# linkedin/ml-ease

Hardware: NVIDIA H100
Metric: ADMM iterations/sec (higher is better)
Workload: dtype f32 data / f64 reductions / bf16 (dense) or e4m3 (CSR) Gram operands

## Files before the change

ml-ease_b200/csrc/k3_cholesky.cu:

```cuda
#include <algorithm>
#include <cstdlib>

#include "kernels.cuh"

namespace mlease {

constexpr int NB = 32;
constexpr int TB = 64;

__global__ void chol_prep_kernel(const Problem* __restrict__ probs, int share) {
  const Problem& pb = probs[blockIdx.z];
  const float* __restrict__ hpart = share > 1 ? probs[blockIdx.z - blockIdx.z % share].Hpart : pb.Hpart;
  Ctrl* c = pb.ctrl;
  if (c->done || !c->need_hess) return;
  const int ldh = pb.ldh, Dt = pb.Dt, Dp = pb.Dp, S = pb.gram_slices;
  const int i = blockIdx.y * blockDim.y + threadIdx.y;
  const int j = blockIdx.x * blockDim.x + threadIdx.x;
  if (i >= ldh || j >= ldh || j > i) return;
  double v;
  if (i < Dt) {
    double s = 0.0;
    const size_t off = (size_t)i * Dp + j;
    for (int t = 0; t < S; t++) s += (double)hpart[(size_t)t * Dp * Dp + off];
    s *= (double)pb.gram_unscale;
    if (i == j) s += pb.q[i];
    v = s;
  } else {
    v = (i == j) ? 1.0 : 0.0;
  }
  pb.Lc[(size_t)i * ldh + j] = v;
}

constexpr int RB = 64;
__global__ void __launch_bounds__(32) chol_diag_kernel(const Problem* __restrict__ probs, int k) {
  const Problem& pb = probs[blockIdx.x];
  Ctrl* c = pb.ctrl;
  if (c->done || !c->need_hess) return;
  __shared__ double A[NB][NB + 1];
  const int ldh = pb.ldh;
  const int c0 = k * NB;
  const double* H = pb.Lc;
  const int lane = threadIdx.x;
  double a[NB];
#pragma unroll
  for (int kk = 0; kk < NB; kk++) a[kk] = (kk <= lane) ? H[(size_t)(c0 + lane) * ldh + c0 + kk] : 0.0;
  int bad = 0;
  double dinv[NB];
#pragma unroll
  for (int j = 0; j < NB; j++) {
    double djj = __shfl_sync(0xffffffffu, a[j], j);
    if (!(djj > 0.0)) { bad = 1; djj = 1.0; }
    const double r = rsqrt(djj);
    dinv[j] = r;
    if (lane == j) a[j] = djj * r;
    else if (lane > j) a[j] = a[j] * r;
#pragma unroll
    for (int kk = j + 1; kk < NB; kk++) {
      const double lkj = __shfl_sync(0xffffffffu, a[j], kk);
      if (lane >= kk) a[kk] -= a[j] * lkj;
    }
  }
#pragma unroll
  for (int kk = 0; kk < NB; kk++) {
    A[lane][kk] = (kk <= lane) ? a[kk] : 0.0;
    pb.Ldiag[(size_t)(c0 + lane) * NB + kk] = (kk <= lane) ? a[kk] : 0.0;
  }
  __syncwarp();
  {
    const int cc = lane;
    double li[NB];
#pragma unroll
    for (int i = 0; i < NB; i++) {
      double sacc = 0.0;
#pragma unroll
      for (int kk = 0; kk < NB; kk++)
        if (kk < i) sacc += A[i][kk] * li[kk];
      li[i] = i < cc ? 0.0 : (i == cc ? dinv[i] : -sacc * dinv[i]);
    }
#pragma unroll
    for (int i = 0; i < NB; i++) pb.Ldinv[(size_t)(c0 + i) * NB + cc] = li[i];
  }
  if (lane == 0 && bad) c->fail = 1;
}

__global__ void __launch_bounds__(256) chol_panel_kernel(const Problem* __restrict__ probs, int k) {
  const Problem& pb = probs[blockIdx.y];
  Ctrl* c = pb.ctrl;
  if (c->done || !c->need_hess) return;
  __shared__ double Li[NB][NB + 1];
  __shared__ double P[RB][NB + 1];
  const int ldh = pb.ldh;
  const int c0 = k * NB;
  double* H = pb.Lc;
  const int tid = threadIdx.x;
  const int r0 = c0 + NB + blockIdx.x * RB;
  if (r0 >= ldh) return;
  const int rows = min(RB, ldh - r0);
  for (int e = tid; e < NB * NB; e += 256) Li[e / NB][e % NB] = pb.Ldinv[(size_t)(c0 + e / NB) * NB + e % NB];
  for (int e = tid; e < rows * NB; e += 256) {
    const int i = e / NB, j = e % NB;
    P[i][j] = H[(size_t)(r0 + i) * ldh + c0 + j];
  }
  __syncthreads();
  for (int e = tid; e < rows * NB; e += 256) {
    const int i = e / NB, j = e % NB;
    double sacc = 0.0;
    for (int kk = 0; kk <= j; kk++) sacc += P[i][kk] * Li[j][kk];
    H[(size_t)(r0 + i) * ldh + c0 + j] = sacc;
  }
}

__global__ void __launch_bounds__(256) chol_update_kernel(const Problem* __restrict__ probs, int k, int jlimit) {
  const Problem& pb = probs[blockIdx.z];
  Ctrl* c = pb.ctrl;
  if (c->done || !c->need_hess) return;
  if (blockIdx.x > blockIdx.y) return;
  const int ldh = pb.ldh;
  const int base = (k + 1) * NB;
  const int i0 = base + blockIdx.y * TB, j0 = base + blockIdx.x * TB;
  if (i0 >= ldh || j0 >= ldh || j0 >= jlimit) return;
  __shared__ double Ai[NB][TB + 2];
  __shared__ double Aj[NB][TB + 2];
  double* H = pb.Lc;
  const int c0 = k * NB;
  const int tid = threadIdx.x;
  for (int e = tid; e < TB * NB; e += 256) {
    const int i = e / NB, kk = e % NB;
    Ai[kk][i] = (i0 + i < ldh) ? H[(size_t)(i0 + i) * ldh + c0 + kk] : 0.0;
    Aj[kk][i] = (j0 + i < ldh) ? H[(size_t)(j0 + i) * ldh + c0 + kk] : 0.0;
  }
  __syncthreads();
  const int ti = (tid / 16) * 4, tj = (tid % 16) * 4;
  double acc[4][4];
#pragma unroll
  for (int a = 0; a < 4; a++)
#pragma unroll
    for (int b = 0; b < 4; b++) acc[a][b] = 0.0;
#pragma unroll 4
  for (int kk = 0; kk < NB; kk++) {
    double x[4], y[4];
#pragma unroll
    for (int a = 0; a < 4; a++) { x[a] = Ai[kk][ti + a]; y[a] = Aj[kk][tj + a]; }
#pragma unroll
    for (int a = 0; a < 4; a++)
#pragma unroll
      for (int b = 0; b < 4; b++) acc[a][b] += x[a] * y[b];
  }
#pragma unroll
  for (int a = 0; a < 4; a++)
#pragma unroll
    for (int b = 0; b < 4; b++) {
      const int i = i0 + ti + a, j = j0 + tj + b;
      if (i < ldh && j <= i && j < jlimit) H[(size_t)i * ldh + j] -= acc[a][b];
    }
}

__global__ void chol_finish_kernel(const Problem* __restrict__ probs) {
  const Problem& pb = probs[blockIdx.y];
  Ctrl* c = pb.ctrl;
  if (c->done || !c->need_hess) return;
  const int c0 = blockIdx.x * NB;
  for (int e = threadIdx.x; e < NB * NB; e += blockDim.x) {
    const int i = e / NB, j = e % NB;
    if (j <= i) pb.Lc[(size_t)(c0 + i) * pb.ldh + c0 + j] = pb.Ldiag[(size_t)(c0 + i) * NB + j];
  }
  if (threadIdx.x == 0 && blockIdx.x == 0) {
    if (c->fail == 1) { c->done = 1; c->hess_valid = 0; }
    else { c->hess_valid = 1; c->hess_builds++; c->tot_hess++; c->bfgs_count = 0; c->h0_scale = 1.0; c->build_step = c->newton_steps; c->ysym_use = pb.Ysym; }
  }
}

template <int NR>
__global__ void __launch_bounds__(256) trinv_kernel(const Problem* __restrict__ probs, int leaf) {
  const Problem& pb = probs[blockIdx.y];
  Ctrl* c = pb.ctrl;
  if (c->done || !c->need_hess) return;
  constexpr int CPT = NR / 8;
  __shared__ double Lt[NB][NB + 1];
  __shared__ double Yt[NB][NR + 2];
  __shared__ double Rb[NB][NR + 2];
  const int ldh = pb.ldh;
  const int c0 = blockIdx.x * NR;
  if (c0 >= ldh) return;
  const int nb = leaf > 0 ? min(ldh, (c0 / leaf + 1) * leaf) / NB : ldh / NB;
  const int ncols = min(NR, ldh - c0);
  const int kb0 = c0 / NB;
  const int tid = threadIdx.x;
  const int ti = tid >> 3, tq = tid & 7;
  const double* __restrict__ L = pb.Lc;
  double* __restrict__ Y = pb.Yinv;
  const int lr = tid >> 3, lc = (tid & 7) * 4;
  for (int kb = kb0; kb < nb; kb++) {
// ... 21 lines not shown
        const double l = Lt[ti][kk];
#pragma unroll
        for (int q = 0; q < CPT; q++) acc[q] -= l * Yt[kk][tq + 8 * q];
      }
      __syncthreads();
    }
#pragma unroll
    for (int q = 0; q < CPT; q++) Rb[ti][tq + 8 * q] = acc[q];
#pragma unroll
    for (int q = 0; q < 4; q++) Lt[lr][lc + q] = pb.Ldinv[(size_t)(r0 + lr) * NB + lc + q];
    __syncthreads();
    double yv[CPT];
#pragma unroll
    for (int q = 0; q < CPT; q++) yv[q] = 0.0;
    for (int kk = 0; kk <= ti; kk++) {
      const double l = Lt[ti][kk];
#pragma unroll
      for (int q = 0; q < CPT; q++) yv[q] += l * Rb[kk][tq + 8 * q];
    }
#pragma unroll
    for (int q = 0; q < CPT; q++)
      if (tq + 8 * q < ncols) Y[(size_t)(r0 + ti) * ldh + c0 + tq + 8 * q] = yv[q];
    __syncthreads();
  }
}

__global__ void __launch_bounds__(256) hinv_syrk_kernel(const Problem* __restrict__ probs) {
  const Problem& pb = probs[blockIdx.z];
  Ctrl* c = pb.ctrl;
  if (c->done || !c->need_hess) return;
  if (blockIdx.x > blockIdx.y) return;
  const int ldh = pb.ldh;
  const int i0 = blockIdx.y * TB, j0 = blockIdx.x * TB;
  if (i0 >= ldh) return;
  __shared__ double Yi[NB][TB + 1];
  __shared__ double Yj[NB][TB + 1];
  const double* Y = pb.Yinv;
  const int tid = threadIdx.x;
  const int ti = (tid / 16) * 4, tj = (tid % 16) * 4;
  double acc[4][4];
#pragma unroll
  for (int a = 0; a < 4; a++)
#pragma unroll
    for (int b = 0; b < 4; b++) acc[a][b] = 0.0;
  for (int k0 = (i0 / NB) * NB; k0 < ldh; k0 += NB) {
    for (int e = tid; e < NB * TB; e += 256) {
      const int kk = e / TB, cc = e % TB;
      const int k = k0 + kk;
      Yi[kk][cc] = (i0 + cc < ldh && i0 + cc <= k) ? Y[(size_t)k * ldh + i0 + cc] : 0.0;
      Yj[kk][cc] = (j0 + cc < ldh && j0 + cc <= k) ? Y[(size_t)k * ldh + j0 + cc] : 0.0;
    }
    __syncthreads();
#pragma unroll 4
    for (int kk = 0; kk < NB; kk++) {
      double x[4], y[4];
#pragma unroll
      for (int a = 0; a < 4; a++) { x[a] = Yi[kk][ti + a]; y[a] = Yj[kk][tj + a]; }
#pragma unroll
      for (int a = 0; a < 4; a++)
#pragma unroll
        for (int b = 0; b < 4; b++) acc[a][b] += x[a] * y[b];
    }
    __syncthreads();
  }
#pragma unroll
  for (int a = 0; a < 4; a++)
#pragma unroll
    for (int b = 0; b < 4; b++) {
      const int i = i0 + ti + a, j = j0 + tj + b;
      if (i < ldh && j < ldh) {
        pb.Hinv[(size_t)i * ldh + j] = acc[a][b];
        pb.Hinv[(size_t)j * ldh + i] = acc[a][b];
      }
    }
}


constexpr int WNB = 256;
constexpr int WLEAF = 256;
constexpr int DM = 128, DN = 64, DK = 16;
constexpr int DA_SZ = DM * 20 > DK * (DM + 4) ? DM * 20 : DK * (DM + 4);
constexpr int DB_SZ = DN * 20 > DK * (DN + 4) ? DN * 20 : DK * (DN + 4);
constexpr size_t DGEMM_SMEM = (size_t)2 * (DA_SZ + DB_SZ) * sizeof(double);

__device__ __forceinline__ void dmma_8x8x4(double& c0, double& c1, double a, double b) {
  asm volatile("mma.sync.aligned.m8n8k4.row.col.f64.f64.f64.f64 {%0,%1}, {%2}, {%3}, {%0,%1};" : "+d"(c0), "+d"(c1) : "d"(a), "d"(b));
}

template <bool A_KC, bool B_KC>
__global__ void __launch_bounds__(256, 2) dgemm_kernel(const Problem* __restrict__ probs, int mode, int p0, int p1) {
  const Problem& pb = probs[blockIdx.z];
  Ctrl* ctl = pb.ctrl;
  if (ctl->done || !ctl->need_hess) return;
  const int ldh = pb.ldh;
  const double* A; const double* B; double* C;
  int M, N, K;
  if (mode == 0) {
    const int c = p0, w = p1;
    M = N = ldh - c - w; K = w;
    A = B = pb.Lc + (size_t)(c + w) * ldh + c;
    C = pb.Lc + (size_t)(c + w) * ldh + (c + w);
  } else if (mode == 1 || mode == 2) {
    const int m = p0, r0 = 2 * blockIdx.y * m;
    const int m2 = min(m, ldh - r0 - m);
    if (m2 <= 0) return;
    M = m2; N = m;
    if (mode == 1) {
      K = m;
      A = pb.Lc + (size_t)(r0 + m) * ldh + r0;
      B = pb.Yinv + (size_t)r0 * ldh + r0;
      C = pb.Hinv + (size_t)(r0 + m) * ldh + r0;
    } else {
      K = m2;
      A = pb.Yinv + (size_t)(r0 + m) * ldh + (r0 + m);
      B = pb.Hinv + (size_t)(r0 + m) * ldh + r0;
      C = pb.Yinv + (size_t)(r0 + m) * ldh + r0;
    }
  } else {
    M = N = K = ldh;
    A = B = pb.Yinv;
    C = pb.Hinv;
  }
  const int tiles_n = (N + DN - 1) / DN;
  const int i0 = (blockIdx.x / tiles_n) * DM, j0 = (blockIdx.x % tiles_n) * DN;
  if (i0 >= M) return;
  if ((mode == 0 || mode == 3) && j0 >= i0 + DM) return;
  int klo = 0, khi = K;
  if (mode == 1) klo = j0;
  if (mode == 2) khi = min(K, i0 + DM);
  if (mode == 3) klo = max(i0, j0);

  extern __shared__ double dg_smem[];
  double* As = dg_smem;
  double* Bs = dg_smem + 2 * DA_SZ;
  const int tid = threadIdx.x, warp = tid >> 5, lane = tid & 31;
  const int g = lane >> 2, tg = lane & 3;
  const int wm = (warp & 3) * 32, wn = (warp >> 2) * 32;

  double2 ra[4], rb[2];
  auto gload = [&](int k0) {
#pragma unroll
    for (int q = 0; q < 4; q++) {
      if (A_KC) {
        const int row = (tid >> 3) + 32 * q, kk = (tid & 7) * 2;
        ra[q] = (i0 + row < M) ? *reinterpret_cast<const double2*>(A + (size_t)(i0 + row) * ldh + k0 + kk) : make_double2(0.0, 0.0);
      } else {
        const int kk = (tid >> 6) + 4 * q, ii = (tid & 63) * 2;
        ra[q] = (i0 + ii < M) ? *reinterpret_cast<const double2*>(A + (size_t)(k0 + kk) * ldh + i0 + ii) : make_double2(0.0, 0.0);
      }
    }
#pragma unroll
    for (int q = 0; q < 2; q++) {
      if (B_KC) {
        const int col = (tid >> 3) + 32 * q, kk = (tid & 7) * 2;
        rb[q] = (j0 + col < N) ? *reinterpret_cast<const double2*>(B + (size_t)(j0 + col) * ldh + k0 + kk) : make_double2(0.0, 0.0);
      } else {
        const int kk = (tid >> 5) + 8 * q, jj = (tid & 31) * 2;
        rb[q] = (j0 + jj < N) ? *reinterpret_cast<const double2*>(B + (size_t)(k0 + kk) * ldh + j0 + jj) : make_double2(0.0, 0.0);
      }
    }
  };
  auto sstore = [&](int buf) {
    double* a = As + buf * DA_SZ;
    double* b = Bs + buf * DB_SZ;
#pragma unroll
    for (int q = 0; q < 4; q++) {
      if (A_KC) *reinterpret_cast<double2*>(a + ((tid >> 3) + 32 * q) * 20 + (tid & 7) * 2) = ra[q];
      else *reinterpret_cast<double2*>(a + ((tid >> 6) + 4 * q) * (DM + 4) + (tid & 63) * 2) = ra[q];
    }
#pragma unroll
    for (int q = 0; q < 2; q++) {
      if (B_KC) *reinterpret_cast<double2*>(b + ((tid >> 3) + 32 * q) * 20 + (tid & 7) * 2) = rb[q];
      else *reinterpret_cast<double2*>(b + ((tid >> 5) + 8 * q) * (DN + 4) + (tid & 31) * 2) = rb[q];
    }
  };

  double acc[4][4][2];
#pragma unroll
  for (int a = 0; a < 4; a++)
#pragma unroll
    for (int b = 0; b < 4; b++) acc[a][b][0] = acc[a][b][1] = 0.0;

  if (klo < khi) {
    gload(klo);
    sstore(0);
    __syncthreads();
    int buf = 0;
    for (int k0 = klo; k0 < khi; k0 += DK) {
      const bool more = k0 + DK < khi;
      if (more) gload(k0 + DK);
      const double* a = As + buf * DA_SZ;
      const double* b = Bs + buf * DB_SZ;
#pragma unroll
      for (int k4 = 0; k4 < DK; k4 += 4) {
        double fa[4], fb[4];
#pragma unroll
        for (int f = 0; f < 4; f++) {
          fa[f] = A_KC ? a[(wm + f * 8 + g) * 20 + k4 + tg] : a[(k4 + tg) * (DM + 4) + wm + f * 8 + g];
          fb[f] = B_KC ? b[(wn + f * 8 + g) * 20 + k4 + tg] : b[(k4 + tg) * (DN + 4) + wn + f * 8 + g];
        }
#pragma unroll
        for (int fm = 0; fm < 4; fm++)
#pragma unroll
          for (int fn = 0; fn < 4; fn++) dmma_8x8x4(acc[fm][fn][0], acc[fm][fn][1], fa[fm], fb[fn]);
      }
      if (more) sstore(buf ^ 1);
      __syncthreads();
      buf ^= 1;
    }
  }

#pragma unroll
  for (int fm = 0; fm < 4; fm++) {
    const int i = i0 + wm + fm * 8 + g;
    if (i >= M) continue;
#pragma unroll
    for (int fn = 0; fn < 4; fn++) {
      const int j = j0 + wn + fn * 8 + 2 * tg;
      if (j >= N) continue;
      const double v0 = acc[fm][fn][0], v1 = acc[fm][fn][1];
      if (mode == 0) {
        double* d = C + (size_t)i * ldh + j;
        if (j + 1 <= i) { double2 o = *reinterpret_cast<double2*>(d); o.x -= v0; o.y -= v1; *reinterpret_cast<double2*>(d) = o; }
        else if (j <= i) d[0] -= v0;
      } else if (mode == 1) {
        *reinterpret_cast<double2*>(C + (size_t)i * ldh + j) = make_double2(v0, v1);
      } else if (mode == 2) {
        *reinterpret_cast<double2*>(C + (size_t)i * ldh + j) = make_double2(-v0, -v1);
      } else {
        if (j <= i) { C[(size_t)i * ldh + j] = v0; C[(size_t)j * ldh + i] = v0; }
        if (j + 1 <= i) { C[(size_t)i * ldh + j + 1] = v1; C[(size_t)(j + 1) * ldh + i] = v1; }
      }
    }
  }
}

template <bool A_KC, bool B_KC>
static cudaError_t dgemm_launch(const Problem* d_probs, int nprob, int mode, int p0, int p1, int M, int N, int nmerge, cudaStream_t st,
                                int* launches) {
  {
    static bool configured[64] = {};
    int dev = 0;
    cudaGetDevice(&dev);
    if (dev < 0 || dev >= 64 || !configured[dev]) {
      cudaError_t e = cudaFuncSetAttribute(dgemm_kernel<A_KC, B_KC>, cudaFuncAttributeMaxDynamicSharedMemorySize, (int)DGEMM_SMEM);
      if (e != cudaSuccess) return e;
      if (dev >= 0 && dev < 64) configured[dev] = true;
    }
  }
  const int tiles = ((M + DM - 1) / DM) * ((N + DN - 1) / DN);
  if (tiles <= 0 || nmerge <= 0) return cudaSuccess;
  dgemm_kernel<A_KC, B_KC><<<dim3(tiles, nmerge, nprob), 256, DGEMM_SMEM, st>>>(d_probs, mode, p0, p1);
  if (launches) *launches += 1;
  return cudaGetLastError();
}

constexpr int TM = 128, TN = 128, TK = 16;
constexpr int TA_LD = TK + 4, TB_LD = TN + 8;
constexpr int TA_SZ = TM * TA_LD, TB_SZ = TK * TB_LD;

__device__ __forceinline__ uint32_t to_tf32(double x) {
  uint32_t r;
  const float f = (float)x;
  asm("cvt.rna.tf32.f32 %0, %1;" : "=r"(r) : "f"(f));
  return r;
}
__device__ __forceinline__ void mma_tf32_16x8x8(float (&c)[4], const uint32_t (&a)[4], const uint32_t (&b)[2]) {
  asm volatile("mma.sync.aligned.m16n8k8.row.col.f32.tf32.tf32.f32 {%0,%1,%2,%3}, {%4,%5,%6,%7}, {%8,%9}, {%0,%1,%2,%3};"
               : "+f"(c[0]), "+f"(c[1]), "+f"(c[2]), "+f"(c[3])
               : "r"(a[0]), "r"(a[1]), "r"(a[2]), "r"(a[3]), "r"(b[0]), "r"(b[1]));
}

__global__ void __launch_bounds__(256, 2) merge_tf32_kernel(const Problem* __restrict__ probs, int mode, int m) {
  const Problem& pb = probs[blockIdx.z];
  Ctrl* ctl = pb.ctrl;
  if (ctl->done || !ctl->need_hess) return;
  const int ldh = pb.ldh;
  const int r0 = 2 * blockIdx.y * m;
  const int m2 = min(m, ldh - r0 - m);
  if (m2 <= 0) return;
  const int M = m2, N = m;
  const double* __restrict__ A; const double* __restrict__ B; double* __restrict__ C;
  int K;
  if (mode == 1) {
    K = m;
    A = pb.Lc + (size_t)(r0 + m) * ldh + r0;
    B = pb.Yinv + (size_t)r0 * ldh + r0;
    C = pb.Hinv + (size_t)(r0 + m) * ldh + r0;
  } else {
    K = m2;
    A = pb.Yinv + (size_t)(r0 + m) * ldh + (r0 + m);
    B = pb.Hinv + (size_t)(r0 + m) * ldh + r0;
    C = pb.Yinv + (size_t)(r0 + m) * ldh + r0;
  }
  const int tiles_n = (N + TN - 1) / TN;
  const int i0 = (blockIdx.x / tiles_n) * TM, j0 = (blockIdx.x % tiles_n) * TN;
  if (i0 >= M) return;
  int klo = 0, khi = K;
  if (mode == 1) klo = j0;
  else khi = min(K, i0 + TM);

  __shared__ __align__(16) uint32_t As[2][TA_SZ];
  __shared__ __align__(16) uint32_t Bs[2][TB_SZ];
  const int tid = threadIdx.x, warp = tid >> 5, lane = tid & 31;
  const int g = lane >> 2, tg = lane & 3;
  const int wm = (warp & 1) * 64, wn = (warp >> 1) * 32;

  const double* pa = A + (size_t)(i0 + (tid >> 3)) * ldh + klo + (tid & 7) * 2;
  const double* pbk = B + (size_t)(klo + (tid >> 6)) * ldh + j0 + (tid & 63) * 2;
  const size_t a_step = (size_t)32 * ldh, b_step = (size_t)4 * ldh, b_adv = (size_t)TK * ldh;
  unsigned a_ok = 0;
#pragma unroll
  for (int q = 0; q < 4; q++) a_ok |= (i0 + (tid >> 3) + 32 * q < M ? 1u : 0u) << q;
  const bool b_ok = j0 + (tid & 63) * 2 < N;
  double2 ra[4], rb[4];
  auto gload = [&]() {
#pragma unroll
    for (int q = 0; q < 4; q++)
      ra[q] = ((a_ok >> q) & 1u) ? __ldg(reinterpret_cast<const double2*>(pa + q * a_step)) : make_double2(0.0, 0.0);
#pragma unroll
    for (int q = 0; q < 4; q++)
      rb[q] = b_ok ? __ldg(reinterpret_cast<const double2*>(pbk + q * b_step)) : make_double2(0.0, 0.0);
    pa += TK;
    pbk += b_adv;
  };
  auto sstore = [&](int buf) {
#pragma unroll
    for (int q = 0; q < 4; q++) {
      const int row = (tid >> 3) + 32 * q, kk = (tid & 7) * 2;
      *reinterpret_cast<uint2*>(&As[buf][row * TA_LD + kk]) = make_uint2(to_tf32(ra[q].x), to_tf32(ra[q].y));
    }
#pragma unroll
    for (int q = 0; q < 4; q++) {
      const int kk = (tid >> 6) + 4 * q, jj = (tid & 63) * 2;
      *reinterpret_cast<uint2*>(&Bs[buf][kk * TB_LD + jj]) = make_uint2(to_tf32(rb[q].x), to_tf32(rb[q].y));
    }
// ... 12 lines not shown
    sstore(0);
    __syncthreads();
    int buf = 0;
    for (int k0 = klo; k0 < khi; k0 += TK) {
      const bool more = k0 + TK < khi;
      if (more) gload();
      const uint32_t* a = As[buf];
      const uint32_t* b = Bs[buf];
#pragma unroll
      for (int k8 = 0; k8 < TK; k8 += 8) {
        uint32_t fa[4][4], fb[4][2];
#pragma unroll
        for (int f = 0; f < 4; f++) {
          const uint32_t* pa = a + (wm + f * 16 + g) * TA_LD + k8 + tg;
          fa[f][0] = pa[0];
          fa[f][1] = pa[8 * TA_LD];
          fa[f][2] = pa[4];
          fa[f][3] = pa[8 * TA_LD + 4];
          const uint32_t* pbk = b + (k8 + tg) * TB_LD + wn + f * 8 + g;
          fb[f][0] = pbk[0];
          fb[f][1] = pbk[4 * TB_LD];
        }
#pragma unroll
        for (int fm = 0; fm < 4; fm++)
#pragma unroll
          for (int fn = 0; fn < 4; fn++) mma_tf32_16x8x8(acc[fm][fn], fa[fm], fb[fn]);
      }
      if (more) sstore(buf ^ 1);
      __syncthreads();
      buf ^= 1;
    }
  }

  const double sgn = mode == 1 ? 1.0 : -1.0;
#pragma unroll
  for (int fm = 0; fm < 4; fm++)
#pragma unroll
    for (int h = 0; h < 2; h++) {
      const int i = i0 + wm + fm * 16 + g + 8 * h;
      if (i >= M) continue;
#pragma unroll
      for (int fn = 0; fn < 4; fn++) {
        const int j = j0 + wn + fn * 8 + 2 * tg;
        if (j >= N) continue;
        *reinterpret_cast<double2*>(C + (size_t)i * ldh + j) =
            make_double2(sgn * (double)acc[fm][fn][2 * h], sgn * (double)acc[fm][fn][2 * h + 1]);
      }
    }
}

static cudaError_t merge_tf32_launch(const Problem* d_probs, int nprob, int mode, int m, int nmerge, cudaStream_t st, int* launches) {
  const int t = (m + TM - 1) / TM;
  if (t <= 0 || nmerge <= 0) return cudaSuccess;
  merge_tf32_kernel<<<dim3(t * ((m + TN - 1) / TN), nmerge, nprob), 256, 0, st>>>(d_probs, mode, m);
  if (launches) *launches += 1;
  return cudaGetLastError();
}
constexpr int CHOL_WIDE_MIN = 1000;

__global__ void __launch_bounds__(256) ysym_kernel(const Problem* __restrict__ probs) {
  const Problem& pb = probs[blockIdx.z];
  const Ctrl* c = pb.ctrl;
  if (c->done || !c->need_hess) return;
  const int bi = blockIdx.y, bj = blockIdx.x;
  if (bj > bi) return;
  __shared__ float t[32][33];
  const int ldh = pb.ldh;
  const int tx = threadIdx.x & 31, ty = threadIdx.x >> 5;
  for (int r = ty; r < 32; r += 8) {
    const int i = bi * 32 + r, j = bj * 32 + tx;
    const float v = j <= i ? (float)pb.Yinv[(size_t)i * ldh + j] : 0.f;
    t[r][tx] = v;
    if (j <= i) pb.Ysym[(size_t)i * ldh + j] = __float2bfloat16_rn(v);
  }
  __syncthreads();
  for (int r = ty; r < 32; r += 8) {
    const int j = bj * 32 + r, i = bi * 32 + tx;
    if (j < i) pb.Ysym[(size_t)j * ldh + i] = __float2bfloat16_rn(t[tx][r]);
  }
}

bool cholesky_factored_direction(int ldh) { return ldh > 2048; }

static cudaError_t cholesky_launch_wide(const Problem* d_probs, int nprob, int ldh, cudaStream_t st, int* launches, bool factored_direction) {
  cudaError_t e;
  for (int c = 0; c < ldh; c += WNB) {
    const int w = std::min(WNB, ldh - c);
    for (int k = c / NB; k < (c + w) / NB; k++) {
      const int below = ldh - (k + 1) * NB;
      const int gx = below > 0 ? (below + RB - 1) / RB : 1;
      chol_diag_kernel<<<nprob, 32, 0, st>>>(d_probs, k);
      if (below > 0) chol_panel_kernel<<<dim3(gx, nprob), 256, 0, st>>>(d_probs, k);
      if (launches) *launches += 2;
      const int inner = c + w - (k + 1) * NB;
      if (inner > 0) {
        chol_update_kernel<<<dim3((inner + TB - 1) / TB, (below + TB - 1) / TB, nprob), 256, 0, st>>>(d_probs, k, c + w);
        if (launches) *launches += 1;
      }
    }
    const int rest = ldh - c - w;
    if (rest > 0 && (e = dgemm_launch<true, true>(d_probs, nprob, 0, c, w, rest, rest, 1, st, launches)) != cudaSuccess) return e;
  }
  trinv_kernel<64><<<dim3((ldh + 63) / 64, nprob), 256, 0, st>>>(d_probs, WLEAF);
  if ((e = cudaGetLastError()) != cudaSuccess) return e;
  if (launches) *launches += 1;
  for (int m = WLEAF; m < ldh; m *= 2) {
    const int nmerge = (ldh + 2 * m - 1) / (2 * m);
    if (factored_direction) {
      if ((e = merge_tf32_launch(d_probs, nprob, 1, m, nmerge, st, launches)) != cudaSuccess) return e;
      if ((e = merge_tf32_launch(d_probs, nprob, 2, m, nmerge, st, launches)) != cudaSuccess) return e;
      continue;
    }
    if ((e = dgemm_launch<true, false>(d_probs, nprob, 1, m, 0, m, m, nmerge, st, launches)) != cudaSuccess) return e;
    if ((e = dgemm_launch<true, false>(d_probs, nprob, 2, m, 0, m, m, nmerge, st, launches)) != cudaSuccess) return e;
  }
  if (factored_direction) {
    ysym_kernel<<<dim3(ldh / 32, ldh / 32, nprob), 256, 0, st>>>(d_probs);
    if (launches) *launches += 1;
    return cudaGetLastError();
  }
  return dgemm_launch<false, false>(d_probs, nprob, 3, 0, 0, ldh, ldh, 1, st, launches);
}

__global__ void chol_share_begin_kernel(const Problem* __restrict__ probs, int nprob, int share) {
  const int b = blockIdx.x * blockDim.x + threadIdx.x;
  if (b < nprob && b % share != 0) probs[b].ctrl->need_hess = 0;
}
__global__ void chol_share_end_kernel(const Problem* __restrict__ probs, int nprob, int share) {
  const int b = blockIdx.x * blockDim.x + threadIdx.x;
  if (b >= nprob || b % share == 0) return;
  Ctrl* c = probs[b].ctrl;
  const Ctrl* lead = probs[b - b % share].ctrl;
  c->need_hess = 1;
  if (lead->fail == 1) { c->fail = 1; c->done = 1; c->hess_valid = 0; }
  else {
    c->hess_valid = 1; c->hess_builds++; c->tot_hess++; c->bfgs_count = 0; c->h0_scale = 1.0; c->build_step = c->newton_steps;
    c->ysym_use = probs[b - b % share].Ysym;
  }
}
__device__ __forceinline__ int detach_owner(const Problem* __restrict__ probs, int nprob, int b) {
  const Problem& pb = probs[b];
  const Ctrl* c = pb.ctrl;
  const void* use = c->ysym_use;
  if (!use || use == (const void*)pb.Ysym || (!c->done && c->need_hess)) return -1;
  for (int j = 0; j < nprob; j++) {
    if ((const void*)probs[j].Ysym != use) continue;
    const Ctrl* oc = probs[j].ctrl;
    return (!oc->done && oc->need_hess) ? j : -1;
  }
  return -1;
}
__global__ void __launch_bounds__(256) ysym_detach_kernel(const Problem* __restrict__ probs, int nprob, int mode) {
  if (mode == 1) {
    const int b = blockIdx.x * blockDim.x + threadIdx.x;
    if (b < nprob && detach_owner(probs, nprob, b) >= 0) probs[b].ctrl->ysym_use = probs[b].Ysym;
    return;
  }
  const int b = blockIdx.y;
  const int o = detach_owner(probs, nprob, b);
  if (o < 0) return;
  const size_t n16 = (size_t)probs[b].ldh * probs[b].ldh / 8;
  const uint4* __restrict__ src = reinterpret_cast<const uint4*>(probs[o].Ysym);
  uint4* __restrict__ dst = reinterpret_cast<uint4*>(probs[b].Ysym);
  for (size_t e = (size_t)blockIdx.x * blockDim.x + threadIdx.x; e < n16; e += (size_t)gridDim.x * blockDim.x) dst[e] = src[e];
}
cudaError_t cholesky_detach_followers(const Problem* d_probs, int nprob, int ldh, cudaStream_t st, int* launches) {
  if (!cholesky_factored_direction(ldh)) return cudaSuccess;
  ysym_detach_kernel<<<dim3(64, nprob), 256, 0, st>>>(d_probs, nprob, 0);
  ysym_detach_kernel<<<(nprob + 255) / 256, 256, 0, st>>>(d_probs, nprob, 1);
  if (launches) *launches += 2;
  return cudaGetLastError();
}

cudaError_t cholesky_share_begin(const Problem* d_probs, int nprob, int share, cudaStream_t st, int* launches) {
  chol_share_begin_kernel<<<(nprob + 127) / 128, 128, 0, st>>>(d_probs, nprob, share);
  if (launches) *launches += 1;
  return cudaGetLastError();
}
cudaError_t cholesky_share_end(const Problem* d_probs, int nprob, int share, cudaStream_t st, int* launches) {
  chol_share_end_kernel<<<(nprob + 127) / 128, 128, 0, st>>>(d_probs, nprob, share);
  if (launches) *launches += 1;
  return cudaGetLastError();
}

cudaError_t cholesky_launch(const Problem* d_probs, int nprob, int ldh, cudaStream_t st, int* launches, int share, int skip_prep, int want_hinv) {
  if (!skip_prep) {
    dim3 blk(32, 8);
    dim3 grd((ldh + 31) / 32, (ldh + 7) / 8, nprob);
    chol_prep_kernel<<<grd, blk, 0, st>>>(d_probs, share);
    if (launches) *launches += 1;
  }
  const int nb = ldh / NB;
  if (ldh > CHOL_WIDE_MIN) {
    cudaError_t e = cholesky_launch_wide(d_probs, nprob, ldh, st, launches, cholesky_factored_direction(ldh) && !want_hinv);
    if (e != cudaSuccess) return e;
  } else {
    for (int k = 0; k < nb; k++) {
      const int below = ldh - (k + 1) * NB;
      const int gx = below > 0 ? (below + RB - 1) / RB : 1;
      chol_diag_kernel<<<nprob, 32, 0, st>>>(d_probs, k);
      if (below > 0) chol_panel_kernel<<<dim3(gx, nprob), 256, 0, st>>>(d_probs, k);
      if (launches) *launches += 2;
      if (below > 0) {
        const int T = (below + TB - 1) / TB;
        chol_update_kernel<<<dim3(T, T, nprob), 256, 0, st>>>(d_probs, k, ldh);
        if (launches) *launches += 1;
      }
    }
    trinv_kernel<32><<<dim3((ldh + 31) / 32, nprob), 256, 0, st>>>(d_probs, 0);
    cudaError_t e = cudaGetLastError();
    if (e != cudaSuccess) return e;
    if (launches) *launches += 1;
    const int T = (ldh + TB - 1) / TB;
    hinv_syrk_kernel<<<dim3(T, T, nprob), 256, 0, st>>>(d_probs);
    if (launches) *launches += 1;
  }
  chol_finish_kernel<<<dim3(nb, nprob), 256, 0, st>>>(d_probs);
  if (launches) *launches += 1;
  return cudaGetLastError();
}

}
```

ml-ease_b200/csrc/kernels.cuh:

```cuda
#pragma once
#include "common.cuh"

namespace mlease {

bool k1_dense_plan(int ldx, int* R_out, int* S_out, int* G_out, size_t* smem_out, int* ctas_per_sm);
int k1_csr_window(int ldx);
cudaError_t k1_launch(const Problem* d_probs, int nprob, bool csr, int ldx, int has_bias, int ctas_per_problem,
                      int force_emit, cudaStream_t stream, int* launches, int csr_fx = 0, int nprob_dyn = 0, int mode = K1_GRAD);

bool k1f_plan(long long n, int ldx, int L, int num_sms, int* S_out, int* rows_out, int* LP_out, size_t* smem_out);
cudaError_t k1f_build(long long n, int Dg, long long nnz, const long long* rowptr, const int* colidx, const float* vals, int S, int sg_rows, int* ngrp_out,
                      int** perm_out, int** depth_out, long long** goff_out, unsigned short** row16_out, float** val_out, long long* total_out,
                      cudaStream_t st);
cudaError_t k1f_launch(const Problem* d_probs, int ngroups, int L, int S, int LP, size_t smem, int has_bias, int force_emit, cudaStream_t st, int* launches,
                       int mode = K1_GRAD);
cudaError_t csr_row_l1_max(long long n, const long long* rowptr, const float* vals, unsigned* out, cudaStream_t st);

cudaError_t newton_begin(const Problem* d_probs, int nprob, double xtol, int max_newton, int hess_policy,
                         int invalidate_hess, int rebuild_is_expensive, cudaStream_t st, int* launches);
cudaError_t k1_reduce_decide(const Problem* d_probs, int nprob, int Dt, cudaStream_t st, int* launches, int spec = 0);
cudaError_t newton_solve(const Problem* d_probs, int nprob, int ldh, cudaStream_t st, int* launches, int group_L = 1);
cudaError_t newton_gemv_tri(const Problem* d_probs, int nprob, int ldh, int group_L, cudaStream_t st);
cudaError_t cg_begin(const Problem* d_probs, int nprob, cudaStream_t st, int* launches);
cudaError_t hv_reduce(const Problem* d_probs, int nprob, int Dt, int out, cudaStream_t st, int* launches);
cudaError_t cg_init(const Problem* d_probs, int nprob, int Dt, cudaStream_t st, int* launches);
cudaError_t cg_step(const Problem* d_probs, int nprob, int Dt, cudaStream_t st, int* launches);
cudaError_t cg_poll(const Problem* d_probs, int nprob, int* d_any, cudaStream_t st, int* launches);
cudaError_t newton_finish(const Problem* d_probs, int nprob, int Dt, cudaStream_t st, int* launches);

int gram_make_tensor_map(void* out_map_host, const void* xt, long long n, int Dp);
int gram_tile_list(int Dp, short* bi_bj_pairs, int max_tiles, int csr_tiles = 0);
cudaError_t gram_launch_wgmma(const Problem* d_probs, int nprob, const void* d_tmaps, const void* d_tiles, int ntiles,
                              int nslices, int force, cudaStream_t st, int* launches, int share = 0);
cudaError_t gram_launch_csr_wgmma(const Problem* d_probs, int nprob, const void* d_tiles, int ntiles, int nslices, int force,
                                  cudaStream_t st, int* launches, int share = 0);
cudaError_t gram_launch_csr_sparse(const Problem* d_probs, int nprob, const void* d_tiles, int ntiles, int force, cudaStream_t st,
                                   int* launches, int share = 0);
long long gram_sparse_max_rows();
__host__ __device__ inline int gram_sparse_span(long long entries, int nblk, long long ngroups) {
  const double per = (double)entries / ((double)(nblk > 1 ? nblk : 1) * (double)(ngroups > 1 ? ngroups : 1));
  const int g = (int)(0.75 * 448 / (per > 1.0 ? per : 1.0));
  return g < 1 ? 1 : (g > 8 ? 8 : g);
}
cudaError_t csr_bm_offsets(long long n, const long long* rowptr, const int* colidx, int bias_col, int nblk, long long ngroups, long long* offs,
                           cudaStream_t st);
cudaError_t csr_bm_fill(long long n, const long long* rowptr, const int* colidx, const float* vals, int bias_col, int nblk, long long ngroups,
                        const long long* offs, unsigned short* keys, float* bvals, cudaStream_t st);
cudaError_t gram_launch_simt(const Problem* d_probs, int nprob, int Dp, int force, cudaStream_t st, int* launches);

cudaError_t cholesky_launch(const Problem* d_probs, int nprob, int ldh, cudaStream_t st, int* launches, int share = 0, int skip_prep = 0,
                            int want_hinv = 0);
bool cholesky_factored_direction(int ldh);
cudaError_t cholesky_share_begin(const Problem* d_probs, int nprob, int share, cudaStream_t st, int* launches);
cudaError_t cholesky_share_end(const Problem* d_probs, int nprob, int share, cudaStream_t st, int* launches);
cudaError_t cholesky_detach_followers(const Problem* d_probs, int nprob, int ldh, cudaStream_t st, int* launches);
cudaError_t admm_reset(const Problem* d_probs, int nprob, int L, double* d_z, int ldv, const double* d_rho_eff,
                       cudaStream_t st, int* launches);
cudaError_t admm_init(const Problem* d_probs, int nprob, const double* d_z, int ldv, cudaStream_t st, int* launches);
cudaError_t admm_pack(const Problem* d_probs, int nlocal_parts, int L, int Dt, double* d_exchange, cudaStream_t st,
                      int* launches);
cudaError_t admm_consensus(const Problem* d_probs, int nlocal_parts, int L, int Dt, int ldv, int P, const double* d_exchange_sum,
                           double* d_z, const double* d_wz, const double* d_rho_eff_next, double* d_diff, cudaStream_t st,
                           int* launches, const double* d_l1_thr = nullptr);

cudaError_t postvar_rowweights(const Problem* d_probs, int nprob, const long long* d_row_start, long long nrows, int has_bias, double* d_dvec,
                               cudaStream_t st, int* launches);
cudaError_t postvar_diag(const Problem* d_probs, int nprob, const long long* d_row_start, long long nrows, const double* d_dvec, int has_bias,
                         cudaStream_t st, int* launches);
cudaError_t postvar_hessian(const Problem* d_prob, bool csr, int ldh, const double* d_dvec, const double* d_q, int has_bias, cudaStream_t st,
                            int* launches);

}
```

Measured before the change: 47.51.

## Overlap Cholesky panel chain with trailing SYRK on a side stream, fuse diag into panel

Fuses the diagonal-block factorisation into the panel kernel, which now runs on a capped grid that loops over rows, cutting one launch per block column. Replaces the trailing-update dgemm with a dedicated SYRK kernel that uses a 3-stage cp.async pipeline and m16n8k4 FP64 MMA. The SYRK is split so the next panel chain runs on a high-priority side stream while the remaining trailing update proceeds on the main stream. The dgemm is also switched to m16n8k4 with a triangular tile map for the symmetric mode. These add stream and event management under a mutex, plus a test kernel for checking MMA shapes.

Measured after the change: 49.36 (median of 6 runs). +3.9%, better.

```diff
diff --git a/ml-ease_b200/csrc/k3_cholesky.cu b/ml-ease_b200/csrc/k3_cholesky.cu
--- a/ml-ease_b200/csrc/k3_cholesky.cu
+++ b/ml-ease_b200/csrc/k3_cholesky.cu
@@ -1,5 +1,6 @@
 #include <algorithm>
 #include <cstdlib>
+#include <mutex>
 
 #include "kernels.cuh"
 
@@ -32,26 +33,22 @@
 }
 
 constexpr int RB = 64;
-__global__ void __launch_bounds__(32) chol_diag_kernel(const Problem* __restrict__ probs, int k) {
-  const Problem& pb = probs[blockIdx.x];
-  Ctrl* c = pb.ctrl;
-  if (c->done || !c->need_hess) return;
-  __shared__ double A[NB][NB + 1];
+constexpr int PANEL_CTAS = 32;
+__device__ __forceinline__ void chol_diag_block(const Problem& pb, int c0, bool store, double (&A)[NB][NB + 1], double (&Li)[NB][NB + 1],
+                                                double (&dinv)[NB]) {
   const int ldh = pb.ldh;
-  const int c0 = k * NB;
   const double* H = pb.Lc;
   const int lane = threadIdx.x;
   double a[NB];
 #pragma unroll
   for (int kk = 0; kk < NB; kk++) a[kk] = (kk <= lane) ? H[(size_t)(c0 + lane) * ldh + c0 + kk] : 0.0;
   int bad = 0;
-  double dinv[NB];
 #pragma unroll
   for (int j = 0; j < NB; j++) {
     double djj = __shfl_sync(0xffffffffu, a[j], j);
     if (!(djj > 0.0)) { bad = 1; djj = 1.0; }
     const double r = rsqrt(djj);
-    dinv[j] = r;
+    if (lane == j) dinv[j] = r;
     if (lane == j) a[j] = djj * r;
     else if (lane > j) a[j] = a[j] * r;
 #pragma unroll
@@ -63,51 +60,62 @@
 #pragma unroll
   for (int kk = 0; kk < NB; kk++) {
     A[lane][kk] = (kk <= lane) ? a[kk] : 0.0;
-    pb.Ldiag[(size_t)(c0 + lane) * NB + kk] = (kk <= lane) ? a[kk] : 0.0;
+    if (store) pb.Ldiag[(size_t)(c0 + lane) * NB + kk] = (kk <= lane) ? a[kk] : 0.0;
   }
   __syncwarp();
   {
     const int cc = lane;
-    double li[NB];
 #pragma unroll
     for (int i = 0; i < NB; i++) {
       double sacc = 0.0;
 #pragma unroll
       for (int kk = 0; kk < NB; kk++)
-        if (kk < i) sacc += A[i][kk] * li[kk];
-      li[i] = i < cc ? 0.0 : (i == cc ? dinv[i] : -sacc * dinv[i]);
-    }
-#pragma unroll
-    for (int i = 0; i < NB; i++) pb.Ldinv[(size_t)(c0 + i) * NB + cc] = li[i];
-  }
-  if (lane == 0 && bad) c->fail = 1;
+        if (kk < i) sacc += A[i][kk] * Li[kk][cc];
+      const double li = i < cc ? 0.0 : (i == cc ? dinv[i] : -sacc * dinv[i]);
+      Li[i][cc] = li;
+      if (store) pb.Ldinv[(size_t)(c0 + i) * NB + cc] = li;
+    }
+  }
+  if (store && lane == 0 && bad) pb.ctrl->fail = 1;
 }
 
 __global__ void __launch_bounds__(256) chol_panel_kernel(const Problem* __restrict__ probs, int k) {
   const Problem& pb = probs[blockIdx.y];
   Ctrl* c = pb.ctrl;
   if (c->done || !c->need_hess) return;
+  __shared__ double A[NB][NB + 1];
   __shared__ double Li[NB][NB + 1];
   __shared__ double P[RB][NB + 1];
+  __shared__ double dinv[NB];
   const int ldh = pb.ldh;
   const int c0 = k * NB;
   double* H = pb.Lc;
   const int tid = threadIdx.x;
-  const int r0 = c0 + NB + blockIdx.x * RB;
-  if (r0 >= ldh) return;
-  const int rows = min(RB, ldh - r0);
-  for (int e = tid; e < NB * NB; e += 256) Li[e / NB][e % NB] = pb.Ldinv[(size_t)(c0 + e / NB) * NB + e % NB];
-  for (int e = tid; e < rows * NB; e += 256) {
-    const int i = e / NB, j = e % NB;
-    P[i][j] = H[(size_t)(r0 + i) * ldh + c0 + j];
-  }
+  const int rfirst = c0 + NB + blockIdx.x * RB;
+  if (tid < 32) chol_diag_block(pb, c0, blockIdx.x == 0, A, Li, dinv);
+  else if (rfirst < ldh)
+    for (int e = tid - 32; e < min(RB, ldh - rfirst) * NB; e += 224) P[e / NB][e % NB] = H[(size_t)(rfirst + e / NB) * ldh + c0 + e % NB];
   __syncthreads();
-  for (int e = tid; e < rows * NB; e += 256) {
-    const int i = e / NB, j = e % NB;
-    double sacc = 0.0;
-    for (int kk = 0; kk <= j; kk++) sacc += P[i][kk] * Li[j][kk];
-    H[(size_t)(r0 + i) * ldh + c0 + j] = sacc;
-  }
+  for (int r0 = rfirst; r0 < ldh; r0 += gridDim.x * RB) {
+    const int rows = min(RB, ldh - r0);
+    if (r0 != rfirst) {
+      __syncthreads();
+      for (int e = tid; e < rows * NB; e += 256) P[e / NB][e % NB] = H[(size_t)(r0 + e / NB) * ldh + c0 + e % NB];
+      __syncthreads();
+    }
+    for (int e = tid; e < rows * NB; e += 256) {
+      const int i = e / NB, j = e % NB;
+      double sacc = 0.0;
+      for (int kk = 0; kk <= j; kk++) sacc += P[i][kk] * Li[j][kk];
+      H[(size_t)(r0 + i) * ldh + c0 + j] = sacc;
+    }
+  }
+}
+static void chol_panel_launch(const Problem* d_probs, int nprob, int ldh, int k, cudaStream_t st, int* launches) {
+  const int below = ldh - (k + 1) * NB;
+  const int gx = below > 0 ? std::min(PANEL_CTAS, (below + RB - 1) / RB) : 1;
+  chol_panel_kernel<<<dim3(gx, nprob), 256, 0, st>>>(d_probs, k);
+  if (launches) *launches += 1;
 }
 
 __global__ void __launch_bounds__(256) chol_update_kernel(const Problem* __restrict__ probs, int k, int jlimit) {
@@ -295,25 +303,40 @@
 constexpr int DA_SZ = DM * 20 > DK * (DM + 4) ? DM * 20 : DK * (DM + 4);
 constexpr int DB_SZ = DN * 20 > DK * (DN + 4) ? DN * 20 : DK * (DN + 4);
 constexpr size_t DGEMM_SMEM = (size_t)2 * (DA_SZ + DB_SZ) * sizeof(double);
+static_assert(DM == 2 * DN, "dgemm_tile: a 128x128 block of a symmetric result is two tiles");
 
 __device__ __forceinline__ void dmma_8x8x4(double& c0, double& c1, double a, double b) {
   asm volatile("mma.sync.aligned.m8n8k4.row.col.f64.f64.f64.f64 {%0,%1}, {%2}, {%3}, {%0,%1};" : "+d"(c0), "+d"(c1) : "d"(a), "d"(b));
 }
+__device__ __forceinline__ void dmma_16x8x4(double& c0, double& c1, double& c2, double& c3, double a0, double a1, double b) {
+  asm volatile("mma.sync.aligned.m16n8k4.row.col.f64.f64.f64.f64 {%0,%1,%2,%3}, {%4,%5}, {%6}, {%0,%1,%2,%3};"
+               : "+d"(c0), "+d"(c1), "+d"(c2), "+d"(c3) : "d"(a0), "d"(a1), "d"(b));
+}
+
+__device__ __forceinline__ bool dgemm_tile(bool tri, int x, int M, int N, int& i0, int& j0) {
+  if (tri) {
+    const int t = x >> 1;
+    int bi = (int)((sqrt(8.0 * t + 1.0) - 1.0) * 0.5);
+    while (bi * (bi + 1) / 2 > t) bi--;
+    while ((bi + 1) * (bi + 2) / 2 <= t) bi++;
+    i0 = bi * DM;
+    j0 = (t - bi * (bi + 1) / 2) * DM + (x & 1) * DN;
+    return j0 < N;
+  }
+  const int tiles_n = (N + DN - 1) / DN;
+  i0 = (x / tiles_n) * DM; j0 = (x % tiles_n) * DN;
+  return i0 < M;
+}
 
 template <bool A_KC, bool B_KC>
-__global__ void __launch_bounds__(256, 2) dgemm_kernel(const Problem* __restrict__ probs, int mode, int p0, int p1) {
+__global__ void __launch_bounds__(256, 2) dgemm_kernel(const Problem* __restrict__ probs, int mode, int p0) {
   const Problem& pb = probs[blockIdx.z];
   Ctrl* ctl = pb.ctrl;
   if (ctl->done || !ctl->need_hess) return;
   const int ldh = pb.ldh;
   const double* A; const double* B; double* C;
   int M, N, K;
-  if (mode == 0) {
-    const int c = p0, w = p1;
-    M = N = ldh - c - w; K = w;
-    A = B = pb.Lc + (size_t)(c + w) * ldh + c;
-    C = pb.Lc + (size_t)(c + w) * ldh + (c + w);
-  } else if (mode == 1 || mode == 2) {
+  if (mode == 1 || mode == 2) {
     const int m = p0, r0 = 2 * blockIdx.y * m;
     const int m2 = min(m, ldh - r0 - m);
     if (m2 <= 0) return;
@@ -334,10 +357,8 @@
     A = B = pb.Yinv;
     C = pb.Hinv;
   }
-  const int tiles_n = (N + DN - 1) / DN;
-  const int i0 = (blockIdx.x / tiles_n) * DM, j0 = (blockIdx.x % tiles_n) * DN;
-  if (i0 >= M) return;
-  if ((mode == 0 || mode == 3) && j0 >= i0 + DM) return;
+  int i0, j0;
+  if (!dgemm_tile(mode == 3, blockIdx.x, M, N, i0, j0)) return;
   int klo = 0, khi = K;
   if (mode == 1) klo = j0;
   if (mode == 2) khi = min(K, i0 + DM);
@@ -413,9 +434,10 @@
           fb[f] = B_KC ? b[(wn + f * 8 + g) * 20 + k4 + tg] : b[(k4 + tg) * (DN + 4) + wn + f * 8 + g];
         }
 #pragma unroll
-        for (int fm = 0; fm < 4; fm++)
-#pragma unroll
-          for (int fn = 0; fn < 4; fn++) dmma_8x8x4(acc[fm][fn][0], acc[fm][fn][1], fa[fm], fb[fn]);
+        for (int fm = 0; fm < 4; fm += 2)
+#pragma unroll
+          for (int fn = 0; fn < 4; fn++)
+            dmma_16x8x4(acc[fm][fn][0], acc[fm][fn][1], acc[fm + 1][fn][0], acc[fm + 1][fn][1], fa[fm], fa[fm + 1], fb[fn]);
       }
       if (more) sstore(buf ^ 1);
       __syncthreads();
@@ -432,11 +454,7 @@
       const int j = j0 + wn + fn * 8 + 2 * tg;
       if (j >= N) continue;
       const double v0 = acc[fm][fn][0], v1 = acc[fm][fn][1];
-      if (mode == 0) {
-        double* d = C + (size_t)i * ldh + j;
-        if (j + 1 <= i) { double2 o = *reinterpret_cast<double2*>(d); o.x -= v0; o.y -= v1; *reinterpret_cast<double2*>(d) = o; }
-        else if (j <= i) d[0] -= v0;
-      } else if (mode == 1) {
+      if (mode == 1) {
         *reinterpret_cast<double2*>(C + (size_t)i * ldh + j) = make_double2(v0, v1);
       } else if (mode == 2) {
         *reinterpret_cast<double2*>(C + (size_t)i * ldh + j) = make_double2(-v0, -v1);
@@ -449,7 +467,7 @@
 }
 
 template <bool A_KC, bool B_KC>
-static cudaError_t dgemm_launch(const Problem* d_probs, int nprob, int mode, int p0, int p1, int M, int N, int nmerge, cudaStream_t st,
+static cudaError_t dgemm_launch(const Problem* d_probs, int nprob, int mode, int p0, int M, int N, int nmerge, cudaStream_t st,
                                 int* launches) {
   {
     static bool configured[64] = {};
@@ -461,10 +479,162 @@
       if (dev >= 0 && dev < 64) configured[dev] = true;
     }
   }
-  const int tiles = ((M + DM - 1) / DM) * ((N + DN - 1) / DN);
+  const int tm = (M + DM - 1) / DM;
+  const int tiles = mode == 3 ? tm * (tm + 1) : tm * ((N + DN - 1) / DN);
   if (tiles <= 0 || nmerge <= 0) return cudaSuccess;
-  dgemm_kernel<A_KC, B_KC><<<dim3(tiles, nmerge, nprob), 256, DGEMM_SMEM, st>>>(d_probs, mode, p0, p1);
+  dgemm_kernel<A_KC, B_KC><<<dim3(tiles, nmerge, nprob), 256, DGEMM_SMEM, st>>>(d_probs, mode, p0);
   if (launches) *launches += 1;
+  return cudaGetLastError();
+}
+
+constexpr int SY_T = 128, SY_TN = 64, SY_LD = DK + 4, SY_STAGES = 3;
+constexpr int SY_WM = 4;
+constexpr int SY_FM = SY_T / SY_WM / 16;
+constexpr int SY_STAGE = (SY_T + SY_TN) * SY_LD;
+constexpr size_t SYRK_SMEM = (size_t)SY_STAGES * SY_STAGE * sizeof(double);
+__device__ __forceinline__ void cp_async16(double* dst, const double* src, bool ok) {
+  asm volatile("cp.async.cg.shared.global [%0], [%1], 16, %2;" ::"r"((uint32_t)__cvta_generic_to_shared(dst)), "l"(src), "r"(ok ? 16 : 0)
+               : "memory");
+}
+__global__ void __launch_bounds__(256, 2) syrk_kernel(const Problem* __restrict__ probs, int c, int w, int off, int n) {
+  const Problem& pb = probs[blockIdx.z];
+  Ctrl* ctl = pb.ctrl;
+  if (ctl->done || !ctl->need_hess) return;
+  const int ldh = pb.ldh, o = c + w + off, M = ldh - o, N = n;
+  int i0, j0;
+  if (M == N) {
+    const int t = blockIdx.x / (SY_T / SY_TN);
+    int bi = (int)((sqrt(8.0 * t + 1.0) - 1.0) * 0.5);
+    while (bi * (bi + 1) / 2 > t) bi--;
+    while ((bi + 1) * (bi + 2) / 2 <= t) bi++;
+    i0 = bi * SY_T; j0 = (t - bi * (bi + 1) / 2) * SY_T + (blockIdx.x % (SY_T / SY_TN)) * SY_TN;
+    if (j0 >= N) return;
+  } else {
+    const int tn = (N + SY_TN - 1) / SY_TN;
+    i0 = (blockIdx.x / tn) * SY_T; j0 = (blockIdx.x % tn) * SY_TN;
+    if (j0 >= i0 + SY_T) return;
+  }
+  const double* A = pb.Lc + (size_t)o * ldh + c;
+  double* C = pb.Lc + (size_t)o * ldh + o;
+  extern __shared__ __align__(16) double sy_smem[];
+  const int tid = threadIdx.x, warp = tid >> 5, lane = tid & 31;
+  const int g = lane >> 2, tg = lane & 3;
+  const int wm = (warp % SY_WM) * (SY_T / SY_WM), wn = (warp / SY_WM) * 32;
+  const int sr = tid >> 3, sk = (tid & 7) * 2;
+  auto issue = [&](int kc) {
+    if (kc < w / DK) {
+      double* st = sy_smem + (kc % SY_STAGES) * SY_STAGE;
+#pragma unroll
+      for (int q = 0; q < SY_T / 32; q++) {
+        const int r = sr + 32 * q;
+        const bool oka = i0 + r < M;
+        cp_async16(st + r * SY_LD + sk, A + (size_t)(oka ? i0 + r : 0) * ldh + kc * DK + sk, oka);
+      }
+#pragma unroll
+      for (int q = 0; q < SY_TN / 32; q++) {
+        const int r = sr + 32 * q;
+        const bool okb = j0 + r < N;
+        cp_async16(st + (SY_T + r) * SY_LD + sk, A + (size_t)(okb ? j0 + r : 0) * ldh + kc * DK + sk, okb);
+      }
+    }
+    asm volatile("cp.async.commit_group;" ::: "memory");
+  };
+  for (int e = tid; e < SY_T * (SY_TN / 16); e += 256) {
+    const int r = e / (SY_TN / 16), q = e % (SY_TN / 16);
+    if (i0 + r < M && j0 + q * 16 < N && j0 + q * 16 <= i0 + r)
+      asm volatile("prefetch.global.L2 [%0];" ::"l"(C + (size_t)(i0 + r) * ldh + j0 + q * 16));
+  }
+  double acc[SY_FM][4][4];
+#pragma unroll
+  for (int a = 0; a < SY_FM; a++)
+#pragma unroll
+    for (int b = 0; b < 4; b++)
+#pragma unroll
+      for (int e = 0; e < 4; e++) acc[a][b][e] = 0.0;
+  issue(0);
+  issue(1);
+  for (int kc = 0; kc < w / DK; kc++) {
+    asm volatile("cp.async.wait_group 1;" ::: "memory");
+    __syncthreads();
+    issue(kc + 2);
+    const double* a = sy_smem + (kc % SY_STAGES) * SY_STAGE;
+    const double* b = a + SY_T * SY_LD;
+#pragma unroll
+    for (int k4 = 0; k4 < DK; k4 += 4) {
+      double fa[SY_FM][2], fb[4];
+#pragma unroll
+      for (int f = 0; f < SY_FM; f++) {
+        fa[f][0] = a[(wm + f * 16 + g) * SY_LD + k4 + tg];
+        fa[f][1] = a[(wm + f * 16 + 8 + g) * SY_LD + k4 + tg];
+      }
+#pragma unroll
+      for (int f = 0; f < 4; f++) fb[f] = b[(wn + f * 8 + g) * SY_LD + k4 + tg];
+#pragma unroll
+      for (int fm = 0; fm < SY_FM; fm++)
+#pragma unroll
+        for (int fn = 0; fn < 4; fn++)
+          dmma_16x8x4(acc[fm][fn][0], acc[fm][fn][1], acc[fm][fn][2], acc[fm][fn][3], fa[fm][0], fa[fm][1], fb[fn]);
+    }
+  }
+  asm volatile("cp.async.wait_group 0;" ::: "memory");
+#pragma unroll
+  for (int fm = 0; fm < SY_FM; fm++)
+#pragma unroll
+    for (int h = 0; h < 2; h++) {
+      const int i = i0 + wm + fm * 16 + 8 * h + g;
+      if (i >= M) continue;
+#pragma unroll
+      for (int fn = 0; fn < 4; fn++) {
+        const int j = j0 + wn + fn * 8 + 2 * tg;
+        if (j >= N) continue;
+        const double v0 = acc[fm][fn][2 * h], v1 = acc[fm][fn][2 * h + 1];
+        double* d = C + (size_t)i * ldh + j;
+        if (j + 1 <= i) { double2 x = *reinterpret_cast<double2*>(d); x.x -= v0; x.y -= v1; *reinterpret_cast<double2*>(d) = x; }
+        else if (j <= i) d[0] -= v0;
+      }
+    }
+}
+static cudaError_t syrk_launch(const Problem* d_probs, int nprob, int c, int w, int off, int n, int M, cudaStream_t st, int* launches) {
+  {
+    static bool configured[64] = {};
+    int dev = 0;
+    cudaGetDevice(&dev);
+    if (dev < 0 || dev >= 64 || !configured[dev]) {
+      cudaError_t e = cudaFuncSetAttribute(syrk_kernel, cudaFuncAttributeMaxDynamicSharedMemorySize, (int)SYRK_SMEM);
+      if (e != cudaSuccess) return e;
+      if (dev >= 0 && dev < 64) configured[dev] = true;
+    }
+  }
+  const int tm = (M + SY_T - 1) / SY_T;
+  const int tiles = M == n ? tm * (tm + 1) / 2 * (SY_T / SY_TN) : tm * ((n + SY_TN - 1) / SY_TN);
+  if (tiles <= 0) return cudaSuccess;
+  syrk_kernel<<<dim3(tiles, 1, nprob), 256, SYRK_SMEM, st>>>(d_probs, c, w, off, n);
+  if (launches) *launches += 1;
+  return cudaGetLastError();
+}
+
+__global__ void __launch_bounds__(32) dmma_shapes_kernel(const double* __restrict__ A, const double* __restrict__ B, int K,
+                                                         double* __restrict__ D8, double* __restrict__ D16) {
+  const int t = blockIdx.x, g = threadIdx.x >> 2, tg = threadIdx.x & 3;
+  const double* a = A + (size_t)t * 16 * K;
+  const double* b = B + (size_t)t * 8 * K;
+  double p[4] = {0.0, 0.0, 0.0, 0.0}, q[4] = {0.0, 0.0, 0.0, 0.0};
+  for (int k = 0; k < K; k += 4) {
+    const double a0 = a[g * K + k + tg], a1 = a[(g + 8) * K + k + tg], bb = b[g * K + k + tg];
+    dmma_8x8x4(p[0], p[1], a0, bb);
+    dmma_8x8x4(p[2], p[3], a1, bb);
+    dmma_16x8x4(q[0], q[1], q[2], q[3], a0, a1, bb);
+  }
+  for (int h = 0; h < 2; h++)
+    for (int e = 0; e < 2; e++) {
+      const size_t o = (size_t)t * 128 + (g + 8 * h) * 8 + 2 * tg + e;
+      D8[o] = p[2 * h + e];
+      D16[o] = q[2 * h + e];
+    }
+}
+cudaError_t dmma_shapes(const double* A, const double* B, int n, int K, double* D8, double* D16, cudaStream_t st) {
+  if (n <= 0 || K <= 0 || K % 4) return cudaErrorInvalidValue;
+  dmma_shapes_kernel<<<n, 32, 0, st>>>(A, B, K, D8, D16);
   return cudaGetLastError();
 }
 
@@ -643,24 +813,63 @@
 
 bool cholesky_factored_direction(int ldh) { return ldh > 2048; }
 
+struct ChainStream {
+  cudaStream_t s = nullptr;
+  cudaEvent_t fork = nullptr, join = nullptr;
+};
+static std::mutex chain_mu;
+static cudaError_t chain_stream(ChainStream** out) {
+  static ChainStream per_dev[64];
+  int dev = 0;
+  cudaError_t e = cudaGetDevice(&dev);
+  if (e != cudaSuccess) return e;
+  if (dev < 0 || dev >= 64) return cudaErrorInvalidDevice;
+  ChainStream& cs = per_dev[dev];
+  if (!cs.s) {
+    int lo = 0, hi = 0;
+    if ((e = cudaDeviceGetStreamPriorityRange(&lo, &hi)) != cudaSuccess) return e;
+    if ((e = cudaEventCreateWithFlags(&cs.fork, cudaEventDisableTiming)) != cudaSuccess) return e;
+    if ((e = cudaEventCreateWithFlags(&cs.join, cudaEventDisableTiming)) != cudaSuccess) return e;
+    if ((e = cudaStreamCreateWithPriority(&cs.s, cudaStreamNonBlocking, hi)) != cudaSuccess) return e;
+  }
+  *out = &cs;
+  return cudaSuccess;
+}
+
+static cudaError_t panel_chain(const Problem* d_probs, int nprob, int ldh, int c, int w, cudaStream_t st, int* launches) {
+  for (int k = c / NB; k < (c + w) / NB; k++) {
+    chol_panel_launch(d_probs, nprob, ldh, k, st, launches);
+    const int below = ldh - (k + 1) * NB;
+    const int inner = c + w - (k + 1) * NB;
+    if (inner > 0) {
+      chol_update_kernel<<<dim3((inner + TB - 1) / TB, (below + TB - 1) / TB, nprob), 256, 0, st>>>(d_probs, k, c + w);
+      if (launches) *launches += 1;
+    }
+  }
+  return cudaGetLastError();
+}
+
 static cudaError_t cholesky_launch_wide(const Problem* d_probs, int nprob, int ldh, cudaStream_t st, int* launches, bool factored_direction) {
   cudaError_t e;
-  for (int c = 0; c < ldh; c += WNB) {
-    const int w = std::min(WNB, ldh - c);
-    for (int k = c / NB; k < (c + w) / NB; k++) {
-      const int below = ldh - (k + 1) * NB;
-      const int gx = below > 0 ? (below + RB - 1) / RB : 1;
-      chol_diag_kernel<<<nprob, 32, 0, st>>>(d_probs, k);
-      if (below > 0) chol_panel_kernel<<<dim3(gx, nprob), 256, 0, st>>>(d_probs, k);
-      if (launches) *launches += 2;
-      const int inner = c + w - (k + 1) * NB;
-      if (inner > 0) {
-        chol_update_kernel<<<dim3((inner + TB - 1) / TB, (below + TB - 1) / TB, nprob), 256, 0, st>>>(d_probs, k, c + w);
-        if (launches) *launches += 1;
-      }
-    }
-    const int rest = ldh - c - w;
-    if (rest > 0 && (e = dgemm_launch<true, true>(d_probs, nprob, 0, c, w, rest, rest, 1, st, launches)) != cudaSuccess) return e;
+  {
+    std::lock_guard<std::mutex> lock(chain_mu);
+    ChainStream* cs = nullptr;
+    if ((e = chain_stream(&cs)) != cudaSuccess) return e;
+    if ((e = panel_chain(d_probs, nprob, ldh, 0, std::min(WNB, ldh), st, launches)) != cudaSuccess) return e;
+    for (int c = 0; c + WNB < ldh; c += WNB) {
+      const int w = WNB, rest = ldh - c - w, nw = std::min(WNB, rest);
+      if ((e = syrk_launch(d_probs, nprob, c, w, 0, nw, rest, st, launches)) != cudaSuccess) return e;
+      if (rest == nw) {
+        if ((e = panel_chain(d_probs, nprob, ldh, c + w, nw, st, launches)) != cudaSuccess) return e;
+        continue;
+      }
+      if ((e = cudaEventRecord(cs->fork, st)) != cudaSuccess) return e;
+      if ((e = cudaStreamWaitEvent(cs->s, cs->fork, 0)) != cudaSuccess) return e;
+      if ((e = panel_chain(d_probs, nprob, ldh, c + w, nw, cs->s, launches)) != cudaSuccess) return e;
+      if ((e = cudaEventRecord(cs->join, cs->s)) != cudaSuccess) return e;
+      if ((e = syrk_launch(d_probs, nprob, c, w, nw, rest - nw, rest - nw, st, launches)) != cudaSuccess) return e;
+      if ((e = cudaStreamWaitEvent(st, cs->join, 0)) != cudaSuccess) return e;
+    }
   }
   trinv_kernel<64><<<dim3((ldh + 63) / 64, nprob), 256, 0, st>>>(d_probs, WLEAF);
   if ((e = cudaGetLastError()) != cudaSuccess) return e;
@@ -672,15 +881,15 @@
       if ((e = merge_tf32_launch(d_probs, nprob, 2, m, nmerge, st, launches)) != cudaSuccess) return e;
       continue;
     }
-    if ((e = dgemm_launch<true, false>(d_probs, nprob, 1, m, 0, m, m, nmerge, st, launches)) != cudaSuccess) return e;
-    if ((e = dgemm_launch<true, false>(d_probs, nprob, 2, m, 0, m, m, nmerge, st, launches)) != cudaSuccess) return e;
+    if ((e = dgemm_launch<true, false>(d_probs, nprob, 1, m, m, m, nmerge, st, launches)) != cudaSuccess) return e;
+    if ((e = dgemm_launch<true, false>(d_probs, nprob, 2, m, m, m, nmerge, st, launches)) != cudaSuccess) return e;
   }
   if (factored_direction) {
     ysym_kernel<<<dim3(ldh / 32, ldh / 32, nprob), 256, 0, st>>>(d_probs);
     if (launches) *launches += 1;
     return cudaGetLastError();
   }
-  return dgemm_launch<false, false>(d_probs, nprob, 3, 0, 0, ldh, ldh, 1, st, launches);
+  return dgemm_launch<false, false>(d_probs, nprob, 3, 0, ldh, ldh, 1, st, launches);
 }
 
 __global__ void chol_share_begin_kernel(const Problem* __restrict__ probs, int nprob, int share) {
@@ -758,10 +967,7 @@
   } else {
     for (int k = 0; k < nb; k++) {
       const int below = ldh - (k + 1) * NB;
-      const int gx = below > 0 ? (below + RB - 1) / RB : 1;
-      chol_diag_kernel<<<nprob, 32, 0, st>>>(d_probs, k);
-      if (below > 0) chol_panel_kernel<<<dim3(gx, nprob), 256, 0, st>>>(d_probs, k);
-      if (launches) *launches += 2;
+      chol_panel_launch(d_probs, nprob, ldh, k, st, launches);
       if (below > 0) {
         const int T = (below + TB - 1) / TB;
         chol_update_kernel<<<dim3(T, T, nprob), 256, 0, st>>>(d_probs, k, ldh);
diff --git a/ml-ease_b200/csrc/kernels.cuh b/ml-ease_b200/csrc/kernels.cuh
--- a/ml-ease_b200/csrc/kernels.cuh
+++ b/ml-ease_b200/csrc/kernels.cuh
@@ -50,6 +50,7 @@
 
 cudaError_t cholesky_launch(const Problem* d_probs, int nprob, int ldh, cudaStream_t st, int* launches, int share = 0, int skip_prep = 0,
                             int want_hinv = 0);
+cudaError_t dmma_shapes(const double* A, const double* B, int n, int K, double* D8, double* D16, cudaStream_t st);
 bool cholesky_factored_direction(int ldh);
 cudaError_t cholesky_share_begin(const Problem* d_probs, int nprob, int share, cudaStream_t st, int* launches);
 cudaError_t cholesky_share_end(const Problem* d_probs, int nprob, int share, cudaStream_t st, int* launches);
```
